# QualityMinds/cistgcn

Measured on AMD Instinct MI355X. Metric: sequences/sec (fwd+bwd) H3.6M 22-joint 50->25, higher is better.
Workload: dtype f32; 1 GPU; cistgcn64_b256_t50_v22; C=64, per_gpu_batch=256, global_batch=256, T_in=50, T_out=25, V=22, parallelism=dp1, graph=True, graph_branches=True, capture_kept=median, mixed_batches=False

## Files before the change

cistgcn_amd/csrc/stgcn_domain_planes.hip:

```cpp
#include "cg_common.h"
#include "stgcn_domain.h"
#include <stdlib.h>

HIP_DYNAMIC_SHARED(unsigned char, cg_dyn_lds)

typedef float cg_f32x4 __attribute__((vector_size(16)));
typedef float cg_f32x2 __attribute__((vector_size(8)));

#define CG_DOMP_THREADS 256
#define CG_DOMP_NW (CG_DOMP_THREADS / 64)

__device__ __forceinline__ int cg_domp_swz(int o) { const int h = o >> 1; return (h & 3) | ((h & 4) << 1); }

template <int VW>
__device__ __forceinline__ void cg_domp_ld(const float* __restrict__ p, bool ok, float (&v)[VW]) {
  if constexpr (VW == 4) {
    cg_f32x4 t = cg_f32x4{0.f, 0.f, 0.f, 0.f};
    if (ok) t = *reinterpret_cast<const cg_f32x4*>(p);
#pragma unroll
    for (int i = 0; i < VW; ++i) v[i] = t[i];
  } else if constexpr (VW == 2) {
    cg_f32x2 t = cg_f32x2{0.f, 0.f};
    if (ok) t = *reinterpret_cast<const cg_f32x2*>(p);
#pragma unroll
    for (int i = 0; i < VW; ++i) v[i] = t[i];
  } else {
    v[0] = ok ? p[0] : 0.f;
  }
}
template <int VW>
__device__ __forceinline__ void cg_domp_st(float* __restrict__ p, const float (&v)[VW]) {
  if constexpr (VW == 4) *reinterpret_cast<cg_f32x4*>(p) = cg_f32x4{v[0], v[1], v[2], v[3]};
  else if constexpr (VW == 2) *reinterpret_cast<cg_f32x2*>(p) = cg_f32x2{v[0], v[1]};
  else p[0] = v[0];
}

template <int DOMAIN>
__device__ __forceinline__ void cg_domp_split(const CgDomP& g, int p, int& grp, int& j) {
  const int t = (int)cg_div((unsigned)p, g.magicV), v = p - t * g.V;
  if (DOMAIN == 0) { grp = v; j = t; } else { grp = t; j = v; }
}

template <int DOMAIN, int VW>
__device__ __forceinline__ void cg_domp_mix_planes(const CgDomP& g, const float* __restrict__ xb, long long cs, int Cin, int KS,
                                                   const float* sW, int WS, float* sZ, int pbeg, int pend, int jshift) {
  const int lane = threadIdx.x & 63, wave = __builtin_amdgcn_readfirstlane(threadIdx.x >> 6), l15 = lane & 15, slot = lane >> 4;
  const int nunits = (pend - pbeg + 16 * VW - 1) / (16 * VW);
  const float* wrow = sW + l15 * WS + slot;
  for (int u = wave; u < nunits; u += CG_DOMP_NW) {
    const int p0 = pbeg + u * 16 * VW + VW * l15;
    const bool pok = p0 < pend;
    const float* xp = xb + p0 + (long long)slot * cs;
    cg_f32x4 acc[VW];
#pragma unroll
    for (int i = 0; i < VW; ++i) acc[i] = cg_f32x4{0.f, 0.f, 0.f, 0.f};
    float xa[4][VW], xc[4][VW];
    auto ld = [&](int k0, float (&xv)[4][VW]) {
#pragma unroll
      for (int s = 0; s < 4; ++s) cg_domp_ld<VW>(xp + (long long)(4 * (k0 + s)) * cs, pok && 4 * (k0 + s) + slot < Cin, xv[s]);
    };
    auto mm = [&](int k0, const float (&xv)[4][VW]) {
#pragma unroll
      for (int s = 0; s < 4; ++s) {
        if (k0 + s >= KS) break;
        const float a = wrow[4 * (k0 + s)];
#pragma unroll
        for (int i = 0; i < VW; ++i) acc[i] = __builtin_amdgcn_mfma_f32_16x16x4f32(a, xv[s][i], acc[i], 0, 0, 0);
      }
    };
    ld(0, xa);
    for (int k0 = 0; k0 < KS; k0 += 8) {
      if (k0 + 4 < KS) ld(k0 + 4, xc);
      mm(k0, xa);
      if (k0 + 4 < KS) {
        if (k0 + 8 < KS) ld(k0 + 8, xa);
        mm(k0 + 4, xc);
      }
    }
    if (pok) {
#pragma unroll
      for (int i = 0; i < VW; ++i) {
        int grp, j;
        cg_domp_split<DOMAIN>(g, p0 + i, grp, j);
        float* dst = sZ + grp * g.GSTR + (j - jshift) + 4 * slot * g.JS;
#pragma unroll
        for (int r = 0; r < 4; ++r) dst[r * g.JS] = acc[i][r];
      }
    }
  }
}

template <int DOMAIN, int VW, int VWB, int NL>
__global__ __launch_bounds__(CG_DOMP_THREADS, 2) void cg_stgcn_planes_fwd_kernel(const float* __restrict__ x, const float* __restrict__ adj,
                                                                 const float* __restrict__ W, const float* __restrict__ bias,
                                                                 float* __restrict__ y, double* __restrict__ ystats, CgDomP g) {
  float* sZ = reinterpret_cast<float*>(cg_dyn_lds);
  float* sW = sZ + g.zfloats;
  double* sStat = reinterpret_cast<double*>(sW + 16 * g.WS);
  const int tid = threadIdx.x, lane = tid & 63, wave = __builtin_amdgcn_readfirstlane(tid >> 6), l15 = lane & 15, slot = lane >> 4;
  const int xcd = blockIdx.x & 7, s = blockIdx.x >> 3;
  const int sb = s / g.NOC, oc = s - sb * g.NOC, b = sb * 8 + xcd;
  if (b >= g.B) return;
  const int o0 = oc * 16;

  for (int e = tid; e < 16 * g.WS; e += CG_DOMP_THREADS) {
    const int o = e / g.WS, c = e - o * g.WS;
    sW[e] = (o0 + o < g.Cout && c < g.Cin) ? W[(long long)(o0 + o) * g.Cin + c] : 0.f;
  }
  if (tid < 32) sStat[tid] = 0.0;
  __syncthreads();

  cg_domp_mix_planes<DOMAIN, VW>(g, x + (long long)b * g.Cin * g.TV, g.TV, g.Cin, g.KS, sW, g.WS, sZ, 0, g.TV, 0);
  __syncthreads();

  const int J = g.J;
  float bv[4];
#pragma unroll
  for (int r = 0; r < 4; ++r) { const int co = o0 + 4 * slot + r; bv[r] = (bias && co < g.Cout) ? bias[co] : 0.f; }
  double st1[4] = {0.0, 0.0, 0.0, 0.0}, st2[4] = {0.0, 0.0, 0.0, 0.0};
  for (int gi = wave; gi < g.NG; gi += CG_DOMP_NW) {
    float gs1[4] = {0.f, 0.f, 0.f, 0.f}, gs2[4] = {0.f, 0.f, 0.f, 0.f};
    const float* ag = adj + ((long long)b * g.NG + gi) * J * J;
    float* zs = sZ + gi * g.GSTR;
    const float* za = zs + l15 * g.JS + slot;
    cg_f32x4 acc[NL * VWB];
#pragma unroll
    for (int i = 0; i < NL * VWB; ++i) acc[i] = cg_f32x4{0.f, 0.f, 0.f, 0.f};
    float ba[4][NL][VWB], bc[4][NL][VWB];
    auto ld = [&](int k0, float (&v)[4][NL][VWB]) {
#pragma unroll
      for (int s2 = 0; s2 < 4; ++s2) {
        const int jr = 4 * (k0 + s2) + slot;
#pragma unroll
        for (int m = 0; m < NL; ++m) {
          const int q0 = (m * 16 + l15) * VWB;
          cg_domp_ld<VWB>(ag + (long long)jr * J + q0, jr < J && q0 < J, v[s2][m]);
        }
      }
    };
    auto mm = [&](int k0, const float (&v)[4][NL][VWB]) {
#pragma unroll
      for (int s2 = 0; s2 < 4; ++s2) {
        if (k0 + s2 >= g.JSTEPS) break;
        const int jr = 4 * (k0 + s2) + slot;
        const float a = jr < J ? za[4 * (k0 + s2)] : 0.f;
#pragma unroll
        for (int m = 0; m < NL; ++m)
#pragma unroll
          for (int i = 0; i < VWB; ++i) acc[m * VWB + i] = __builtin_amdgcn_mfma_f32_16x16x4f32(a, v[s2][m][i], acc[m * VWB + i], 0, 0, 0);
      }
    };
    ld(0, ba);
    for (int k0 = 0; k0 < g.JSTEPS; k0 += 8) {
      if (k0 + 4 < g.JSTEPS) ld(k0 + 4, bc);
      mm(k0, ba);
// ... 372 lines not shown
      cg_f32x4 c0 = cg_f32x4{0.f, 0.f, 0.f, 0.f};
      const float* ap = sdZ + l15 * XS + 4 * slot;
      const float* bp = sX + (16 * wct + l15) * XS + 4 * slot;
      for (int kc = wks; kc < NPT; kc += nks) {
        cg_f32x4 a0 = *reinterpret_cast<const cg_f32x4*>(ap + 16 * kc);
        const cg_f32x4 b0 = *reinterpret_cast<const cg_f32x4*>(bp + 16 * kc);
        if (16 * kc + 16 > Pn) {
#pragma unroll
          for (int s2 = 0; s2 < 4; ++s2) a0[s2] = (16 * kc + 4 * slot + s2 < Pn) ? a0[s2] : 0.f;
        }
#pragma unroll
        for (int s2 = 0; s2 < 4; ++s2) c0 = __builtin_amdgcn_mfma_f32_16x16x4f32(a0[s2], b0[s2], c0, 0, 0, 0);
      }
      if (wks == 0) dWhold = c0;
      else *reinterpret_cast<cg_f32x4*>(sPart + ((wave - MTc) * 64 + lane) * 4) = c0;
    }
    {
      const int ct = wave % MTc;
      const float* ap = sW + slot * WS + 16 * ct + l15;
      float aw[4];
#pragma unroll
      for (int st = 0; st < 4; ++st) aw[st] = ap[4 * st * WS];
#pragma unroll
      for (int i = 0; i < NDX; ++i) {
        const int id = wave + CG_DOMPB_NW * i;
        if (id < ndx) {
          const float* bp = sdZ + slot * XS + 16 * (id / MTc) + l15;
#pragma unroll
          for (int st = 0; st < 4; ++st) dxacc[i] = __builtin_amdgcn_mfma_f32_16x16x4f32(aw[st], bp[4 * st * XS], dxacc[i], 0, 0, 0);
        }
        if ((i & 3) == 3) __builtin_amdgcn_sched_barrier(0);
      }
    }
  }

  const int l15 = l15_, slot = slot_;
  CG_STAMP();
  __syncthreads();
  CG_STAMP();
  dw_flush(g.NOC - 1);
#pragma unroll
  for (int i = 0; i < NDX; ++i) {
    const int id = wave + CG_DOMPB_NW * i;
    if (id < ndx) {
      const int pt = id / MTc, ct = id - pt * MTc;
      float* dst = sX + (16 * ct + 4 * slot) * XS + 16 * pt + l15;
      if (16 * pt + l15 < Pn) {
#pragma unroll
        for (int r = 0; r < 4; ++r) dst[r * XS] = dxacc[i][r];
      }
    }
  }
#pragma unroll
  for (int a = 0; a < NJW; ++a) {
    const int v = wave + CG_DOMPB_NW * a;
    if (v < V) {
#pragma unroll
      for (int qc = 0; qc < 4; ++qc) {
        const int q = 16 * qc + l15;
        if (qc < NQC && q < T) {
          float* db_ = dadj + (((long long)b * V + v) * T + t0) * T;
#pragma unroll
          for (int r = 0; r < 4; ++r) {
            const int t = 4 * slot + r;
            if (t < TCn) db_[t * T + q] = dAacc[a][qc][r];
          }
        }
      }
    }
  }
  __syncthreads();
  {
    float* dxb = dx + (long long)b * Cin * TV + (long long)t0 * V;
    const int nvp = Pn / VWP;
    for (int c0 = 4 * wave; c0 < Cin; c0 += 4 * CG_DOMPB_NW) {
      float xr[8][VWP];
#pragma unroll
      for (int u = 0; u < 8; ++u) {
        const int c = c0 + (u >> 1), i = lane + 64 * (u & 1);
        if (c < Cin && i < nvp) {
          if constexpr (VWP == 4) {
            const cg_f32x4 t = *reinterpret_cast<const cg_f32x4*>(sX + c * XS + i * VWP);
#pragma unroll
            for (int jj = 0; jj < VWP; ++jj) xr[u][jj] = t[jj];
          } else {
#pragma unroll
            for (int jj = 0; jj < VWP; ++jj) xr[u][jj] = sX[c * XS + i * VWP + jj];
          }
        }
      }
#pragma unroll
      for (int u = 0; u < 8; ++u) {
        const int c = c0 + (u >> 1), i = lane + 64 * (u & 1);
        if (c < Cin && i < nvp) cg_domp_st<VWP>(dxb + ((long long)c * TV + i * VWP), xr[u]);
      }
    }
  }
  CG_STAMP();
  CG_STAMP_END();
}

static int cg_domp_up(int v, int m) { return (v + m - 1) / m * m; }

int cg_domp_geom(CgDomP& g, int B, int Cin, int Cout, int T, int V, int domain) {
  if (B <= 0 || Cin <= 0 || Cout <= 0 || T <= 0 || V <= 0 || (domain != 0 && domain != 1)) return CG_ESHAPE;
  g.B = B; g.Cin = Cin; g.Cout = Cout; g.T = T; g.V = V; g.TV = T * V;
  g.NG = domain == 1 ? T : V;
  g.J = domain == 1 ? V : T;
  if (g.J > 64 || Cin > 128 || (long long)T * V > (1 << 20)) return CG_ESHAPE;
  g.JS = g.J + ((2 - g.J) & 3);
  g.GSTR = 16 * g.JS + 2;
  g.NOC = (Cout + 15) / 16;
  g.KS = (Cin + 3) / 4;
  g.WS = 4 * cg_domp_up(g.KS, 4) + 2;
  g.JSTEPS = (g.J + 3) / 4;
  g.zfloats = cg_domp_up(g.NG * g.GSTR + 16, 4);
  g.VW = (g.TV % 4 == 0) ? 4 : (g.TV % 2 == 0) ? 2 : 1;
  if (g.J <= 16) { g.VWB = 1; g.NL = 1; }
  else if (g.J <= 32) { if (g.J % 2 == 0) { g.VWB = 2; g.NL = 1; } else { g.VWB = 1; g.NL = 2; } }
  else { if (g.J % 4 == 0) { g.VWB = 4; g.NL = 1; } else if (g.J % 2 == 0) { g.VWB = 2; g.NL = 2; } else { g.VWB = 1; g.NL = 4; } }
  g.magicV = cg_div_magic(V);
  g.magicNQ = cg_div_magic(g.TV / g.VW);
  return CG_OK;
}

size_t cg_domp_fwd_lds_bytes(const CgDomP& g) { return ((size_t)g.zfloats + 16 * (size_t)g.WS) * sizeof(float) + 32 * sizeof(double); }

int cg_domp_fwd_launch(const float* x, const float* adj, const float* W, const float* bias, float* y, double* ystats,
                       int B, int Cin, int Cout, int T, int V, int domain, hipStream_t stream) {
  CgDomP g;
  int st = cg_domp_geom(g, B, Cin, Cout, T, V, domain);
  if (st != CG_OK) return st;
  const size_t lds = cg_domp_fwd_lds_bytes(g);
  if (lds > 160 * 1024 - 512) return CG_ESHAPE;
  dim3 grid((unsigned)(8 * ((B + 7) / 8) * g.NOC)), block(CG_DOMP_THREADS);
#define CG_DOMP_FWD(D, VW_, VWB_, NL_)                                                                                              \
  if (domain == D && g.VW == VW_ && g.VWB == VWB_ && g.NL == NL_) {                                                               \
    hipError_t e = cg_lds_limit((const void*)cg_stgcn_planes_fwd_kernel<D, VW_, VWB_, NL_>,                                \
                                       lds);                                       \
    if (e != hipSuccess) return (int)e;                                                                                             \
    hipLaunchKernelGGL((cg_stgcn_planes_fwd_kernel<D, VW_, VWB_, NL_>), grid, block, lds, stream, x, adj, W, bias, y, ystats, g);   \
    return cg_launch_status();                                                                                                      \
  }
  CG_DOMP_FWD(0, 4, 2, 2)
  CG_DOMP_FWD(0, 2, 2, 2)
  CG_DOMP_FWD(0, 4, 1, 1)
  CG_DOMP_FWD(0, 2, 1, 1)
  CG_DOMP_FWD(1, 4, 2, 1)
  CG_DOMP_FWD(1, 2, 1, 2)
#undef CG_DOMP_FWD
  return CG_ESHAPE;
}

#define CG_DOMPT_THREADS 512
#define CG_DOMPT_NW 8

template <int VWP, int VWA>
__global__ __launch_bounds__(CG_DOMPT_THREADS, 2) void cg_stgcn_planes_bwd_time_kernel(const float* __restrict__ x, const float* __restrict__ adj,
                                                                       const float* __restrict__ W, const float* __restrict__ dy,
                                                                       float* __restrict__ dx, float* __restrict__ dadj,
                                                                       float* __restrict__ ws, int replicas, CgDomP g) {
  const int T = g.T, V = g.V, Cin = g.Cin, Cout = g.Cout, XS = g.XS, WS = g.WS, CinR = g.CinR, CoR = 16 * g.NOC;
  const int DR = max(CinR, CoR);
  float* sX = reinterpret_cast<float*>(cg_dyn_lds);
  float* sDY = sX + CinR * XS;
  float* sZ = sDY + DR * XS;
  float* sW = sZ + CoR * XS;
  float* sdb = sW + CoR * WS;
  const int tid = threadIdx.x, lane = tid & 63, wave = __builtin_amdgcn_readfirstlane(tid >> 6), l15 = lane & 15, slot = lane >> 4;
  const int xcd = blockIdx.x & 7, sidx = blockIdx.x >> 3;
  const int sb = sidx / g.NTC, tc = sidx - sb * g.NTC, b = sb * 8 + xcd;
  if (b >= g.B) return;
  const int t0 = tc * g.TC, TCn = min(g.TC, T - t0), Pn = TCn * V, NPT = (Pn + 15) / 16;
  const long long TV = g.TV;
  const int MTc = CinR / 16, MTo = g.NOC;

  int nst = 0; (void)nst;
  CG_STAMP();
  {
    const int nvp = Pn / VWP;
    const float* xb = x + (long long)b * Cin * TV + (long long)t0 * V;
    const float* yb = dy + (long long)b * Cout * TV + (long long)t0 * V;
    const int rows = Cin + Cout;
    float buf[16][VWP];
    const int r0 = 16 * wave;
#pragma unroll
    for (int u = 0; u < 16; ++u) {
      const int r = r0 + u;
      const float* src = r < Cin ? xb + (long long)r * TV : yb + (long long)(r - Cin) * TV;
      cg_domp_ld<VWP>(src + lane * VWP, r < rows && lane < nvp, buf[u]);
    }
    const int padc = XS - Pn, nrow = CinR + DR + CoR;
    for (int e = tid; e < nrow * padc; e += CG_DOMPT_THREADS) {
      const int r = e / padc, c = e - r * padc;
      sX[r * XS + Pn + c] = 0.f;
    }
    for (int e = tid; e < (CinR - Cin) * Pn; e += CG_DOMPT_THREADS) sX[Cin * XS + (e / Pn) * XS + e % Pn] = 0.f;
    for (int e = tid; e < (DR - Cout) * Pn; e += CG_DOMPT_THREADS) sDY[Cout * XS + (e / Pn) * XS + e % Pn] = 0.f;
    for (int e = tid; e < CoR * (WS + 1); e += CG_DOMPT_THREADS) sW[e] = 0.f;
    __syncthreads();
    CG_STAMP();
#pragma unroll
    for (int u = 0; u < 16; ++u) {
      const int r = r0 + u;
      float* dst = r < Cin ? sX + r * XS : sDY + (r - Cin) * XS;
      if (r < rows && lane < nvp) {
#pragma unroll
        for (int jj = 0; jj < VWP; ++jj) dst[lane * VWP + jj] = buf[u][jj];
      }
    }
    for (int e = tid; e < Cout * Cin; e += CG_DOMPT_THREADS) {
      const int o = e / Cin, c = e - o * Cin;
      sW[o * WS + c] = W[e];
    }
  }
  CG_STAMP();
  __syncthreads();
  CG_STAMP();

  {
    const int OP = (MTo + 1) / 2, nun = OP * NPT;
    for (int u = wave; u < nun; u += CG_DOMPT_NW) {
      const int pt = u / OP, op = u - pt * OP, ot0 = 2 * op, ot1 = ot0 + 1 < MTo ? ot0 + 1 : ot0;
      cg_f32x4 a0 = cg_f32x4{0.f, 0.f, 0.f, 0.f}, a1 = a0;
      const float* ap0 = sW + (16 * ot0 + l15) * WS + slot;
      const float* ap1 = sW + (16 * ot1 + l15) * WS + slot;
      const float* bp = sX + slot * XS + 16 * pt + l15;
      float f0[12], f1[12];
      auto ld = [&](int k0, float (&f)[12]) {
#pragma unroll
        for (int s2 = 0; s2 < 4; ++s2) { f[s2] = ap0[4 * (k0 + s2)]; f[4 + s2] = ap1[4 * (k0 + s2)]; f[8 + s2] = bp[4 * (k0 + s2) * XS]; }
      };
      auto mm = [&](const float (&f)[12]) {
#pragma unroll
        for (int s2 = 0; s2 < 4; ++s2) {
          a0 = __builtin_amdgcn_mfma_f32_16x16x4f32(f[s2], f[8 + s2], a0, 0, 0, 0);
          a1 = __builtin_amdgcn_mfma_f32_16x16x4f32(f[4 + s2], f[8 + s2], a1, 0, 0, 0);
        }
      };
      const int KS4 = CinR / 4;
      ld(0, f0);
      for (int k0 = 0; k0 < KS4; k0 += 8) {
        if (k0 + 4 < KS4) ld(k0 + 4, f1);
        mm(f0);
        if (k0 + 4 < KS4) {
          if (k0 + 8 < KS4) ld(k0 + 8, f0);
          mm(f1);
        }
      }
      if (16 * pt + l15 < Pn) {
#pragma unroll
        for (int r = 0; r < 4; ++r) {
          sZ[(16 * ot0 + 4 * slot + r) * XS + 16 * pt + l15] = a0[r];
          if (ot1 != ot0) sZ[(16 * ot1 + 4 * slot + r) * XS + 16 * pt + l15] = a1[r];
        }
      }
    }
  }
  CG_STAMP();
  __syncthreads();
  CG_STAMP();

  float dbw[4] = {0.f, 0.f, 0.f, 0.f};
  for (int tl = wave; tl < TCn; tl += CG_DOMPT_NW) {
    const int pb = tl * V;
    const int NVT = (V + 15) / 16;
    const float* at = adj + (((long long)b * T + t0 + tl) * V) * V;
    float bv[2][2][4];
#pragma unroll
    for (int kc = 0; kc < 2; ++kc)
#pragma unroll
      for (int j = 0; j < 2; ++j) {
        const int v = 16 * j + l15, w0 = 16 * kc + 4 * slot;
#pragma unroll
        for (int s0 = 0; s0 < 4; s0 += VWA) {
          float tmp[VWA];
          cg_domp_ld<VWA>(at + v * V + w0 + s0, kc < NVT && j < NVT && v < V && w0 + s0 < V, tmp);
#pragma unroll
          for (int q = 0; q < VWA; ++q) bv[kc][j][s0 + q] = tmp[q];
        }
      }
    {
      cg_f32x4 acc[2][2];
#pragma unroll
      for (int i = 0; i < 2; ++i)
#pragma unroll
        for (int j = 0; j < 2; ++j) acc[i][j] = cg_f32x4{0.f, 0.f, 0.f, 0.f};
      const float* zp = sZ + slot * XS + pb + l15;
      const float* yp = sDY + slot * XS + pb + l15;
      float fa[16], fb[16];
      auto ld = [&](int k0, float (&f)[16]) {
#pragma unroll
        for (int s2 = 0; s2 < 4; ++s2)
#pragma unroll
          for (int i = 0; i < 2; ++i) { f[4 * s2 + i] = zp[4 * (k0 + s2) * XS + 16 * i]; f[4 * s2 + 2 + i] = yp[4 * (k0 + s2) * XS + 16 * i]; }
      };
      auto mm = [&](const float (&f)[16]) {
#pragma unroll
        for (int s2 = 0; s2 < 4; ++s2)
#pragma unroll
          for (int i = 0; i < 2; ++i)
#pragma unroll
            for (int j = 0; j < 2; ++j)
              if (i < NVT && j < NVT) acc[i][j] = __builtin_amdgcn_mfma_f32_16x16x4f32(f[4 * s2 + i], f[4 * s2 + 2 + j], acc[i][j], 0, 0, 0);
      };
      const int KS4 = CoR / 4;
      ld(0, fa);
      for (int k0 = 0; k0 < KS4; k0 += 8) {
        if (k0 + 4 < KS4) ld(k0 + 4, fb);
        mm(fa);
        if (k0 + 4 < KS4) {
          if (k0 + 8 < KS4) ld(k0 + 8, fa);
          mm(fb);
        }
      }
      float* da = dadj + (((long long)b * T + t0 + tl) * V) * V;
#pragma unroll
      for (int i = 0; i < 2; ++i)
#pragma unroll
        for (int j = 0; j < 2; ++j) {
          const int w = 16 * j + l15;
          if (i < NVT && j < NVT && w < V) {
#pragma unroll
            for (int r = 0; r < 4; ++r) {
              const int v = 16 * i + 4 * slot + r;
              if (v < V) da[v * V + w] = acc[i][j][r];
            }
          }
        }
    }
    {
      cg_f32x4 acc[4][2];
#pragma unroll
      for (int i = 0; i < 4; ++i)
#pragma unroll
        for (int j = 0; j < 2; ++j) acc[i][j] = cg_f32x4{0.f, 0.f, 0.f, 0.f};
      float dbp[4] = {0.f, 0.f, 0.f, 0.f};
#pragma unroll
      for (int kc = 0; kc < 2; ++kc) {
        if (kc < NVT) {
          const int w0 = 16 * kc + 4 * slot;
          float av[4][4];
#pragma unroll
          for (int i = 0; i < 4; ++i)
#pragma unroll
            for (int s2 = 0; s2 < 4; ++s2) av[i][s2] = (i < MTo && w0 + s2 < V) ? sDY[(16 * i + l15) * XS + pb + w0 + s2] : 0.f;
#pragma unroll
          for (int s2 = 0; s2 < 4; ++s2)
#pragma unroll
            for (int i = 0; i < 4; ++i) {
              dbp[i] += av[i][s2];
#pragma unroll
              for (int j = 0; j < 2; ++j)
                if (i < MTo && j < NVT) acc[i][j] = __builtin_amdgcn_mfma_f32_16x16x4f32(av[i][s2], bv[kc][j][s2], acc[i][j], 0, 0, 0);
            }
        }
      }
#pragma unroll
      for (int i = 0; i < 4; ++i)
#pragma unroll
        for (int j = 0; j < 2; ++j) {
          const int v = 16 * j + l15;
          if (i < MTo && j < NVT && v < V) {
#pragma unroll
            for (int r = 0; r < 4; ++r) sZ[(16 * i + 4 * slot + r) * XS + pb + v] = acc[i][j][r];
          }
        }
#pragma unroll
      for (int i = 0; i < 4; ++i) dbw[i] += dbp[i];
    }
  }
#pragma unroll
  for (int i = 0; i < 4; ++i) {
    float sdbp = dbw[i];
    sdbp += __shfl_xor(sdbp, 16, 64);
    sdbp += __shfl_xor(sdbp, 32, 64);
    if (i < MTo && slot == 0) atomicAdd(&sdb[16 * i + l15], sdbp);
  }
  CG_STAMP();
  __syncthreads();
  CG_STAMP();

  {
    const int CP = (MTc + 1) / 2, nun = CP * NPT;
    for (int u = wave; u < nun; u += CG_DOMPT_NW) {
      const int pt = u / CP, cp = u - pt * CP, ct0 = 2 * cp, ct1 = ct0 + 1 < MTc ? ct0 + 1 : ct0;
      cg_f32x4 a0 = cg_f32x4{0.f, 0.f, 0.f, 0.f}, a1 = a0;
      const float* ap0 = sW + slot * WS + 16 * ct0 + l15;
      const float* ap1 = sW + slot * WS + 16 * ct1 + l15;
      const float* bp = sZ + slot * XS + 16 * pt + l15;
      float f0[12], f1[12];
      auto ld = [&](int k0, float (&f)[12]) {
#pragma unroll
        for (int s2 = 0; s2 < 4; ++s2) { f[s2] = ap0[4 * (k0 + s2) * WS]; f[4 + s2] = ap1[4 * (k0 + s2) * WS]; f[8 + s2] = bp[4 * (k0 + s2) * XS]; }
      };
      auto mm = [&](const float (&f)[12]) {
#pragma unroll
        for (int s2 = 0; s2 < 4; ++s2) {
          a0 = __builtin_amdgcn_mfma_f32_16x16x4f32(f[s2], f[8 + s2], a0, 0, 0, 0);
          a1 = __builtin_amdgcn_mfma_f32_16x16x4f32(f[4 + s2], f[8 + s2], a1, 0, 0, 0);
        }
      };
      const int KS4 = CoR / 4;
      ld(0, f0);
      for (int k0 = 0; k0 < KS4; k0 += 8) {
        if (k0 + 4 < KS4) ld(k0 + 4, f1);
        mm(f0);
        if (k0 + 4 < KS4) {
          if (k0 + 8 < KS4) ld(k0 + 8, f0);
          mm(f1);
        }
      }
      if (16 * pt + l15 < Pn) {
#pragma unroll
        for (int r = 0; r < 4; ++r) {
          sDY[(16 * ct0 + 4 * slot + r) * XS + 16 * pt + l15] = a0[r];
          if (ct1 != ct0) sDY[(16 * ct1 + 4 * slot + r) * XS + 16 * pt + l15] = a1[r];
        }
      }
    }
    float* wsr = ws + (long long)(blockIdx.x % replicas) * ((long long)Cout * Cin + Cout);
    const int CP2 = (MTc + 1) / 2;
    for (int u = wave; u < MTo * CP2; u += CG_DOMPT_NW) {
      const int ot = u / CP2, cp = u - ot * CP2, ct0 = 2 * cp, ct1 = ct0 + 1 < MTc ? ct0 + 1 : ct0;
      cg_f32x4 a0 = cg_f32x4{0.f, 0.f, 0.f, 0.f}, a1 = a0;
      const float* ap = sZ + (16 * ot + l15) * XS + 4 * slot;
      const float* bp0 = sX + (16 * ct0 + l15) * XS + 4 * slot;
      const float* bp1 = sX + (16 * ct1 + l15) * XS + 4 * slot;
      float fa[12], fb[12];
      auto ld = [&](int kc, float (&f)[12]) {
#pragma unroll
        for (int s2 = 0; s2 < 4; ++s2) {
          const bool ok = 16 * kc + 4 * slot + s2 < Pn;
          f[s2] = ok ? ap[16 * kc + s2] : 0.f; f[4 + s2] = bp0[16 * kc + s2]; f[8 + s2] = bp1[16 * kc + s2];
        }
      };
      auto mm = [&](const float (&f)[12]) {
#pragma unroll
        for (int s2 = 0; s2 < 4; ++s2) {
          a0 = __builtin_amdgcn_mfma_f32_16x16x4f32(f[s2], f[4 + s2], a0, 0, 0, 0);
          a1 = __builtin_amdgcn_mfma_f32_16x16x4f32(f[s2], f[8 + s2], a1, 0, 0, 0);
        }
      };
      ld(0, fa);
      for (int kc = 0; kc < NPT; kc += 2) {
        if (kc + 1 < NPT) ld(kc + 1, fb);
        mm(fa);
        if (kc + 1 < NPT) {
          if (kc + 2 < NPT) ld(kc + 2, fa);
          mm(fb);
        }
      }
#pragma unroll
      for (int r = 0; r < 4; ++r) {
        const int co = 16 * ot + 4 * slot + r;
        if (co < Cout && 16 * ct0 + l15 < Cin) atomicAdd(&wsr[(long long)co * Cin + 16 * ct0 + l15], a0[r]);
        if (ct1 != ct0 && co < Cout && 16 * ct1 + l15 < Cin) atomicAdd(&wsr[(long long)co * Cin + 16 * ct1 + l15], a1[r]);
      }
    }
    if (tid < Cout) atomicAdd(&wsr[(long long)Cout * Cin + tid], sdb[tid]);
  }
  CG_STAMP();
  __syncthreads();
  CG_STAMP();
  {
    float* dxb = dx + (long long)b * Cin * TV + (long long)t0 * V;
    const int nvp = Pn / VWP;
    for (int r0 = 8 * wave; r0 < Cin; r0 += 8 * CG_DOMPT_NW) {
      float buf[8][VWP];
#pragma unroll
      for (int u = 0; u < 8; ++u) {
        const int r = r0 + u;
        if (r < Cin && lane < nvp) {
#pragma unroll
          for (int jj = 0; jj < VWP; ++jj) buf[u][jj] = sDY[r * XS + lane * VWP + jj];
        }
      }
#pragma unroll
      for (int u = 0; u < 8; ++u) {
        const int r = r0 + u;
        if (r < Cin && lane < nvp) cg_domp_st<VWP>(dxb + ((long long)r * TV + lane * VWP), buf[u]);
      }
    }
  }
  CG_STAMP();
  CG_STAMP_END();
}

static int cg_domp_xs(int p) { int xs = cg_domp_up(p, 4); return (xs % 8 == 4) ? xs : xs + 4; }

int cg_domp_bwd_geom(CgDomP& g, int B, int Cin, int Cout, int T, int V) {
  int st = cg_domp_geom(g, B, Cin, Cout, T, V, 0);
  if (st != CG_OK) return st;
  if (Cin > 64 || T > 64) return CG_ESHAPE;
  g.CinR = cg_domp_up(Cin, 16);
  g.YS = 16; g.GZ = 16 * 16 + 1; g.GY = 16 * 16 + 1;
  g.zfl = cg_domp_up(V * g.GZ, 4); g.yfl = cg_domp_up(V * g.GY, 4);
  g.WS = cg_domp_up(g.WS, 2);
  const size_t limit = 160 * 1024 - 1024;
  for (int ntc = (T + 15) / 16; ntc <= T; ++ntc) {
    const int tc0 = (T + ntc - 1) / ntc;
    int best = 0, best_al = 0;
    for (int tc = tc0; tc <= 16 && tc <= tc0 + 2; ++tc) {
      if ((long long)(ntc - 1) * tc >= T) continue;
      const int last = T - (ntc - 1) * tc;
      const int al = ((tc * V) % 4 == 0 && (last * V) % 4 == 0 && g.TV % 4 == 0) ? 4 : ((tc * V) % 2 == 0 && (last * V) % 2 == 0 && g.TV % 2 == 0) ? 2 : 1;
      const int xs = cg_domp_xs(tc * V);
      const int dzfl = 16 * xs > g.yfl ? 16 * xs : g.yfl;
      const size_t bytes = ((size_t)g.CinR * xs + dzfl + g.zfl + g.yfl + 16 * (size_t)g.WS + CG_DOMPB_NW * 256 + 64) * sizeof(float);
      if (bytes > limit || (g.CinR / 16) * ((tc * V + 15) / 16) > CG_DOMPB_NDX * CG_DOMPB_NW || tc * V > 128 * al) continue;
      if (al > best_al) { best = tc; best_al = al; }
    }
    if (best) {
      g.NTC = ntc; g.TC = best; g.VWP = best_al;
      g.XS = cg_domp_xs(best * V);
      g.dzfl = 16 * g.XS > g.yfl ? 16 * g.XS : g.yfl;
      g.bwd_floats = g.CinR * g.XS + g.dzfl + g.zfl + g.yfl + 16 * g.WS + CG_DOMPB_NW * 256 + 64;
      const int lastq = T - 16 * ((T + 15) / 16 - 1);
      g.VWY = (g.TV % 4 == 0 && (lastq * V) % 4 == 0) ? 4 : (g.TV % 2 == 0 && (lastq * V) % 2 == 0) ? 2 : 1;
      g.VWA = T % 4 == 0 ? 4 : T % 2 == 0 ? 2 : 1;
      return CG_OK;
    }
  }
  return CG_ESHAPE;
}

int cg_domp_bwd_launch(const float* x, const float* adj, const float* W, const float* dy, float* dx, float* dadj, float* ws,
                       int replicas, int B, int Cin, int Cout, int T, int V, int domain, hipStream_t stream) {
  if (domain != 0) return CG_ESHAPE;
  CgDomP g;
  int st = cg_domp_bwd_geom(g, B, Cin, Cout, T, V);
  if (st != CG_OK) return st;
  const size_t lds = (size_t)g.bwd_floats * sizeof(float);
  const int njw = (V + CG_DOMPB_NW - 1) / CG_DOMPB_NW;
  dim3 grid((unsigned)(8 * ((B + 7) / 8) * g.NTC)), block(CG_DOMPB_THREADS);
  const int pfn = (16 * V / g.VWY + 31) / 32;
  if (CG_DOMPB_NW % (g.CinR / 16) != 0 || 16 * g.WS > 3 * CG_DOMPB_THREADS) return CG_ESHAPE;
  const int ndxw = ((g.CinR / 16) * ((g.TC * V + 15) / 16) + CG_DOMPB_NW - 1) / CG_DOMPB_NW;
#define CG_DOMP_BWD(VWP_, VWY_, VWA_, NJW_, PF_, NDX_)                                                                             \
  if (g.VWP == VWP_ && g.VWY == VWY_ && g.VWA == VWA_ && njw <= NJW_ && pfn <= PF_ && ndxw <= NDX_) {                             \
    hipError_t e = cg_lds_limit((const void*)cg_stgcn_planes_bwd_kernel<VWP_, VWY_, VWA_, NJW_, PF_, NDX_>,                \
                                       lds);                                      \
    if (e != hipSuccess) return (int)e;                                                                                            \
    hipLaunchKernelGGL((cg_stgcn_planes_bwd_kernel<VWP_, VWY_, VWA_, NJW_, PF_, NDX_>), grid, block, lds, stream, x, adj, W, dy,  \
                       dx, dadj, ws, replicas, g);                                                                                 \
    return cg_launch_status();                                                                                                     \
  }
  CG_DOMP_BWD(4, 4, 2, 3, 3, 10)
  CG_DOMP_BWD(2, 2, 2, 4, 7, 6)
#undef CG_DOMP_BWD
  return CG_ESHAPE;
}

int cg_domp_bwd_time_launch(const float* x, const float* adj, const float* W, const float* dy, float* dx, float* dadj, float* ws,
                            int replicas, int B, int Cin, int Cout, int T, int V, hipStream_t stream) {
  CgDomP g;
  int st = cg_domp_geom(g, B, Cin, Cout, T, V, 1);
  if (st != CG_OK) return st;
  if (Cin > 64 || Cout > 64 || V > 32) return CG_ESHAPE;
  g.CinR = cg_domp_up(Cin, 16);
  const int CoR = 16 * g.NOC;
  g.WS = cg_domp_up(g.CinR, 4) + 2;
  g.TC = CG_DOMPT_NW;
  if (g.TC > T) g.TC = T;
  g.NTC = (T + g.TC - 1) / g.TC;
  const int last = T - (g.NTC - 1) * g.TC;
  g.VWP = ((g.TC * V) % 4 == 0 && (last * V) % 4 == 0 && g.TV % 4 == 0) ? 4 : ((g.TC * V) % 2 == 0 && (last * V) % 2 == 0 && g.TV % 2 == 0) ? 2 : 1;
  if (g.TC * V > 64 * g.VWP || Cin + Cout > 16 * CG_DOMPT_NW) return CG_ESHAPE;
  g.VWA = V % 4 == 0 ? 4 : V % 2 == 0 ? 2 : 1;
  g.XS = g.TC * V + ((2 - g.TC * V) & 3);
  if (g.XS < cg_domp_up(g.TC * V, 16)) g.XS += 4 * ((cg_domp_up(g.TC * V, 16) - g.XS + 3) / 4);
  g.bwd_floats = (g.CinR + (g.CinR > CoR ? g.CinR : CoR) + CoR) * g.XS + CoR * (g.WS + 1) + 64;
  const size_t lds = (size_t)g.bwd_floats * sizeof(float);
  if (lds > 160 * 1024 - 512) return CG_ESHAPE;
  dim3 grid((unsigned)(8 * ((B + 7) / 8) * g.NTC)), block(CG_DOMPT_THREADS);
#define CG_DOMP_BWDT(VWP_, VWA_)                                                                                                   \
  if (g.VWP == VWP_ && g.VWA == VWA_) {                                                                                            \
    hipError_t e = cg_lds_limit((const void*)cg_stgcn_planes_bwd_time_kernel<VWP_, VWA_>,                                   \
                                       lds);                                      \
    if (e != hipSuccess) return (int)e;                                                                                            \
    hipLaunchKernelGGL((cg_stgcn_planes_bwd_time_kernel<VWP_, VWA_>), grid, block, lds, stream, x, adj, W, dy, dx, dadj, ws,       \
                       replicas, g);                                                                                               \
    return cg_launch_status();                                                                                                     \
  }
  CG_DOMP_BWDT(4, 2)
  CG_DOMP_BWDT(2, 1)
#undef CG_DOMP_BWDT
  return CG_ESHAPE;
}
```

Baseline: 15220 sequences/sec.

## Double block to 1024 threads, split adjoint/dz work per frame across wave pairs

The backward-time kernel goes from 512 to 1024 threads (16 waves) while keeping an 8-frame time chunk. Each frame now gets two waves, one computing the adjacency gradient and one computing the dz product. Weight staging is restructured so W is loaded into registers early and written into padded LDS in one pass, removing a barrier. A tail-splitting work dealer spreads leftover MFMA tiles across more waves, and the adjacency loads are hoisted ahead of the prologue barrier. The cost is fewer blocks resident per CU (launch bounds drop the min-2-blocks hint), more registers held across phases, and an extra barrier.

```diff
diff --git a/cistgcn_amd/csrc/stgcn_domain_planes.hip b/cistgcn_amd/csrc/stgcn_domain_planes.hip
--- a/cistgcn_amd/csrc/stgcn_domain_planes.hip
+++ b/cistgcn_amd/csrc/stgcn_domain_planes.hip
@@ -1,6 +1,7 @@
 #include "cg_common.h"
 #include "stgcn_domain.h"
 #include <stdlib.h>
+#include <type_traits>
 
 HIP_DYNAMIC_SHARED(unsigned char, cg_dyn_lds)
 
@@ -679,11 +680,32 @@
   return CG_ESHAPE;
 }
 
-#define CG_DOMPT_THREADS 512
-#define CG_DOMPT_NW 8
+#define CG_DOMPT_THREADS 1024
+#define CG_DOMPT_NW 16
+#define CG_DOMPT_TC 8
+#define CG_DOMPT_ROWS 8
+#define CG_DOMPT_WV 5
+static_assert(2 * CG_DOMPT_TC == CG_DOMPT_NW, "P2: two waves per frame of the chunk");
+
+template <class F>
+__device__ __forceinline__ void cg_dompt_deal(int wave, int nun, int NP, int MT, F&& fn) {
+  const int rounds = nun / CG_DOMPT_NW, rem = nun - rounds * CG_DOMPT_NW;
+  const bool split = 2 * rem <= CG_DOMPT_NW;
+  for (int it = 0; it <= rounds; ++it) {
+    int u, half = 0;
+    bool single = false;
+    if (it < rounds) u = wave + it * CG_DOMPT_NW;
+    else if (split) { if (wave >= 2 * rem) break; u = rounds * CG_DOMPT_NW + (wave >> 1); half = wave & 1; single = true; }
+    else { if (wave >= rem) break; u = rounds * CG_DOMPT_NW + wave; }
+    const int outer = u / NP, t0 = 2 * (u - outer * NP) + half;
+    if (t0 >= MT) continue;
+    if (!single && t0 + 1 < MT) fn(outer, t0, std::true_type{});
+    else fn(outer, t0, std::false_type{});
+  }
+}
 
 template <int VWP, int VWA>
-__global__ __launch_bounds__(CG_DOMPT_THREADS, 2) void cg_stgcn_planes_bwd_time_kernel(const float* __restrict__ x, const float* __restrict__ adj,
+__global__ __launch_bounds__(CG_DOMPT_THREADS) void cg_stgcn_planes_bwd_time_kernel(const float* __restrict__ x, const float* __restrict__ adj,
                                                                        const float* __restrict__ W, const float* __restrict__ dy,
                                                                        float* __restrict__ dx, float* __restrict__ dadj,
                                                                        float* __restrict__ ws, int replicas, CgDomP g) {
@@ -702,6 +724,13 @@
   const long long TV = g.TV;
   const int MTc = CinR / 16, MTo = g.NOC;
 
+  const int tl = wave >> 1;
+  const int pb = tl * V;
+  const int NVT = (V + 15) / 16;
+  const bool wave_da = tl < TCn && !(wave & 1), wave_dz = tl < TCn && (wave & 1);
+  const float* at = adj + (((long long)b * T + t0 + tl) * V) * V;
+  float bv[2][2][4];
+
   int nst = 0; (void)nst;
   CG_STAMP();
   {
@@ -709,14 +738,33 @@
     const float* xb = x + (long long)b * Cin * TV + (long long)t0 * V;
     const float* yb = dy + (long long)b * Cout * TV + (long long)t0 * V;
     const int rows = Cin + Cout;
-    float buf[16][VWP];
-    const int r0 = 16 * wave;
-#pragma unroll
-    for (int u = 0; u < 16; ++u) {
+    float buf[CG_DOMPT_ROWS][VWP];
+    const int r0 = CG_DOMPT_ROWS * wave;
+#pragma unroll
+    for (int u = 0; u < CG_DOMPT_ROWS; ++u) {
       const int r = r0 + u;
       const float* src = r < Cin ? xb + (long long)r * TV : yb + (long long)(r - Cin) * TV;
       cg_domp_ld<VWP>(src + lane * VWP, r < rows && lane < nvp, buf[u]);
     }
+    float wv[CG_DOMPT_WV];
+#pragma unroll
+    for (int i = 0; i < CG_DOMPT_WV; ++i) {
+      const int e = tid + i * CG_DOMPT_THREADS, o = e / WS, c = e - o * WS;
+      wv[i] = (o < Cout && c < Cin) ? W[o * Cin + c] : 0.f;
+    }
+#pragma unroll
+    for (int kc = 0; kc < 2; ++kc)
+#pragma unroll
+      for (int j = 0; j < 2; ++j) {
+        const int v = 16 * j + l15, w0 = 16 * kc + 4 * slot;
+#pragma unroll
+        for (int s0 = 0; s0 < 4; s0 += VWA) {
+          float tmp[VWA];
+          cg_domp_ld<VWA>(at + v * V + w0 + s0, wave_dz && kc < NVT && j < NVT && v < V && w0 + s0 < V, tmp);
+#pragma unroll
+          for (int q = 0; q < VWA; ++q) bv[kc][j][s0 + q] = tmp[q];
+        }
+      }
     const int padc = XS - Pn, nrow = CinR + DR + CoR;
     for (int e = tid; e < nrow * padc; e += CG_DOMPT_THREADS) {
       const int r = e / padc, c = e - r * padc;
@@ -724,11 +772,14 @@
     }
     for (int e = tid; e < (CinR - Cin) * Pn; e += CG_DOMPT_THREADS) sX[Cin * XS + (e / Pn) * XS + e % Pn] = 0.f;
     for (int e = tid; e < (DR - Cout) * Pn; e += CG_DOMPT_THREADS) sDY[Cout * XS + (e / Pn) * XS + e % Pn] = 0.f;
-    for (int e = tid; e < CoR * (WS + 1); e += CG_DOMPT_THREADS) sW[e] = 0.f;
-    __syncthreads();
     CG_STAMP();
 #pragma unroll
-    for (int u = 0; u < 16; ++u) {
+    for (int i = 0; i < CG_DOMPT_WV; ++i) {
+      const int e = tid + i * CG_DOMPT_THREADS;
+      if (e < CoR * (WS + 1)) sW[e] = wv[i];
+    }
+#pragma unroll
+    for (int u = 0; u < CG_DOMPT_ROWS; ++u) {
       const int r = r0 + u;
       float* dst = r < Cin ? sX + r * XS : sDY + (r - Cin) * XS;
       if (r < rows && lane < nvp) {
@@ -736,33 +787,34 @@
         for (int jj = 0; jj < VWP; ++jj) dst[lane * VWP + jj] = buf[u][jj];
       }
     }
-    for (int e = tid; e < Cout * Cin; e += CG_DOMPT_THREADS) {
-      const int o = e / Cin, c = e - o * Cin;
-      sW[o * WS + c] = W[e];
-    }
   }
   CG_STAMP();
   __syncthreads();
   CG_STAMP();
 
   {
-    const int OP = (MTo + 1) / 2, nun = OP * NPT;
-    for (int u = wave; u < nun; u += CG_DOMPT_NW) {
-      const int pt = u / OP, op = u - pt * OP, ot0 = 2 * op, ot1 = ot0 + 1 < MTo ? ot0 + 1 : ot0;
+    const int OP = (MTo + 1) / 2;
+    cg_dompt_deal(wave, OP * NPT, OP, MTo, [&](int pt, int ot0, auto two_) {
+      constexpr bool TWO = decltype(two_)::value;
+      const int ot1 = ot0 + 1;
       cg_f32x4 a0 = cg_f32x4{0.f, 0.f, 0.f, 0.f}, a1 = a0;
       const float* ap0 = sW + (16 * ot0 + l15) * WS + slot;
-      const float* ap1 = sW + (16 * ot1 + l15) * WS + slot;
+      const float* ap1 = ap0 + 16 * WS;
       const float* bp = sX + slot * XS + 16 * pt + l15;
       float f0[12], f1[12];
       auto ld = [&](int k0, float (&f)[12]) {
 #pragma unroll
-        for (int s2 = 0; s2 < 4; ++s2) { f[s2] = ap0[4 * (k0 + s2)]; f[4 + s2] = ap1[4 * (k0 + s2)]; f[8 + s2] = bp[4 * (k0 + s2) * XS]; }
+        for (int s2 = 0; s2 < 4; ++s2) {
+          f[s2] = ap0[4 * (k0 + s2)];
+          if constexpr (TWO) f[4 + s2] = ap1[4 * (k0 + s2)];
+          f[8 + s2] = bp[4 * (k0 + s2) * XS];
+        }
       };
       auto mm = [&](const float (&f)[12]) {
 #pragma unroll
         for (int s2 = 0; s2 < 4; ++s2) {
           a0 = __builtin_amdgcn_mfma_f32_16x16x4f32(f[s2], f[8 + s2], a0, 0, 0, 0);
-          a1 = __builtin_amdgcn_mfma_f32_16x16x4f32(f[4 + s2], f[8 + s2], a1, 0, 0, 0);
+          if constexpr (TWO) a1 = __builtin_amdgcn_mfma_f32_16x16x4f32(f[4 + s2], f[8 + s2], a1, 0, 0, 0);
         }
       };
       const int KS4 = CinR / 4;
@@ -779,34 +831,22 @@
 #pragma unroll
         for (int r = 0; r < 4; ++r) {
           sZ[(16 * ot0 + 4 * slot + r) * XS + 16 * pt + l15] = a0[r];
-          if (ot1 != ot0) sZ[(16 * ot1 + 4 * slot + r) * XS + 16 * pt + l15] = a1[r];
-        }
-      }
-    }
+          if constexpr (TWO) sZ[(16 * ot1 + 4 * slot + r) * XS + 16 * pt + l15] = a1[r];
+        }
+      }
+    });
   }
   CG_STAMP();
   __syncthreads();
   CG_STAMP();
 
-  float dbw[4] = {0.f, 0.f, 0.f, 0.f};
-  for (int tl = wave; tl < TCn; tl += CG_DOMPT_NW) {
-    const int pb = tl * V;
-    const int NVT = (V + 15) / 16;
-    const float* at = adj + (((long long)b * T + t0 + tl) * V) * V;
-    float bv[2][2][4];
-#pragma unroll
-    for (int kc = 0; kc < 2; ++kc)
-#pragma unroll
-      for (int j = 0; j < 2; ++j) {
-        const int v = 16 * j + l15, w0 = 16 * kc + 4 * slot;
-#pragma unroll
-        for (int s0 = 0; s0 < 4; s0 += VWA) {
-          float tmp[VWA];
-          cg_domp_ld<VWA>(at + v * V + w0 + s0, kc < NVT && j < NVT && v < V && w0 + s0 < V, tmp);
-#pragma unroll
-          for (int q = 0; q < VWA; ++q) bv[kc][j][s0 + q] = tmp[q];
-        }
-      }
+  cg_f32x4 dz[4][2];
+  float dbp[4] = {0.f, 0.f, 0.f, 0.f};
+#pragma unroll
+  for (int i = 0; i < 4; ++i)
+#pragma unroll
+    for (int j = 0; j < 2; ++j) dz[i][j] = cg_f32x4{0.f, 0.f, 0.f, 0.f};
+  if (wave_da) {
     {
       cg_f32x4 acc[2][2];
 #pragma unroll
@@ -856,13 +896,9 @@
           }
         }
     }
+  }
+  if (wave_dz) {
     {
-      cg_f32x4 acc[4][2];
-#pragma unroll
-      for (int i = 0; i < 4; ++i)
-#pragma unroll
-        for (int j = 0; j < 2; ++j) acc[i][j] = cg_f32x4{0.f, 0.f, 0.f, 0.f};
-      float dbp[4] = {0.f, 0.f, 0.f, 0.f};
 #pragma unroll
       for (int kc = 0; kc < 2; ++kc) {
         if (kc < NVT) {
@@ -879,53 +915,61 @@
               dbp[i] += av[i][s2];
 #pragma unroll
               for (int j = 0; j < 2; ++j)
-                if (i < MTo && j < NVT) acc[i][j] = __builtin_amdgcn_mfma_f32_16x16x4f32(av[i][s2], bv[kc][j][s2], acc[i][j], 0, 0, 0);
+                if (i < MTo && j < NVT) dz[i][j] = __builtin_amdgcn_mfma_f32_16x16x4f32(av[i][s2], bv[kc][j][s2], dz[i][j], 0, 0, 0);
             }
         }
       }
-#pragma unroll
-      for (int i = 0; i < 4; ++i)
-#pragma unroll
-        for (int j = 0; j < 2; ++j) {
-          const int v = 16 * j + l15;
-          if (i < MTo && j < NVT && v < V) {
-#pragma unroll
-            for (int r = 0; r < 4; ++r) sZ[(16 * i + 4 * slot + r) * XS + pb + v] = acc[i][j][r];
-          }
-        }
-#pragma unroll
-      for (int i = 0; i < 4; ++i) dbw[i] += dbp[i];
-    }
-  }
-#pragma unroll
-  for (int i = 0; i < 4; ++i) {
-    float sdbp = dbw[i];
-    sdbp += __shfl_xor(sdbp, 16, 64);
-    sdbp += __shfl_xor(sdbp, 32, 64);
-    if (i < MTo && slot == 0) atomicAdd(&sdb[16 * i + l15], sdbp);
+    }
   }
   CG_STAMP();
   __syncthreads();
   CG_STAMP();
+  if (wave_dz) {
+#pragma unroll
+    for (int i = 0; i < 4; ++i)
+#pragma unroll
+      for (int j = 0; j < 2; ++j) {
+        const int v = 16 * j + l15;
+        if (i < MTo && j < NVT && v < V) {
+#pragma unroll
+          for (int r = 0; r < 4; ++r) sZ[(16 * i + 4 * slot + r) * XS + pb + v] = dz[i][j][r];
+        }
+      }
+#pragma unroll
+    for (int i = 0; i < 4; ++i) {
+      float sdbp = dbp[i];
+      sdbp += __shfl_xor(sdbp, 16, 64);
+      sdbp += __shfl_xor(sdbp, 32, 64);
+      if (i < MTo && slot == 0) atomicAdd(&sdb[16 * i + l15], sdbp);
+    }
+  }
+  CG_STAMP();
+  __syncthreads();
+  CG_STAMP();
 
   {
-    const int CP = (MTc + 1) / 2, nun = CP * NPT;
-    for (int u = wave; u < nun; u += CG_DOMPT_NW) {
-      const int pt = u / CP, cp = u - pt * CP, ct0 = 2 * cp, ct1 = ct0 + 1 < MTc ? ct0 + 1 : ct0;
+    const int CP = (MTc + 1) / 2;
+    cg_dompt_deal(wave, CP * NPT, CP, MTc, [&](int pt, int ct0, auto two_) {
+      constexpr bool TWO = decltype(two_)::value;
+      const int ct1 = ct0 + 1;
       cg_f32x4 a0 = cg_f32x4{0.f, 0.f, 0.f, 0.f}, a1 = a0;
       const float* ap0 = sW + slot * WS + 16 * ct0 + l15;
-      const float* ap1 = sW + slot * WS + 16 * ct1 + l15;
+      const float* ap1 = ap0 + 16;
       const float* bp = sZ + slot * XS + 16 * pt + l15;
       float f0[12], f1[12];
       auto ld = [&](int k0, float (&f)[12]) {
 #pragma unroll
-        for (int s2 = 0; s2 < 4; ++s2) { f[s2] = ap0[4 * (k0 + s2) * WS]; f[4 + s2] = ap1[4 * (k0 + s2) * WS]; f[8 + s2] = bp[4 * (k0 + s2) * XS]; }
+        for (int s2 = 0; s2 < 4; ++s2) {
+          f[s2] = ap0[4 * (k0 + s2) * WS];
+          if constexpr (TWO) f[4 + s2] = ap1[4 * (k0 + s2) * WS];
+          f[8 + s2] = bp[4 * (k0 + s2) * XS];
+        }
       };
       auto mm = [&](const float (&f)[12]) {
 #pragma unroll
         for (int s2 = 0; s2 < 4; ++s2) {
           a0 = __builtin_amdgcn_mfma_f32_16x16x4f32(f[s2], f[8 + s2], a0, 0, 0, 0);
-          a1 = __builtin_amdgcn_mfma_f32_16x16x4f32(f[4 + s2], f[8 + s2], a1, 0, 0, 0);
+          if constexpr (TWO) a1 = __builtin_amdgcn_mfma_f32_16x16x4f32(f[4 + s2], f[8 + s2], a1, 0, 0, 0);
         }
       };
       const int KS4 = CoR / 4;
@@ -942,31 +986,33 @@
 #pragma unroll
         for (int r = 0; r < 4; ++r) {
           sDY[(16 * ct0 + 4 * slot + r) * XS + 16 * pt + l15] = a0[r];
-          if (ct1 != ct0) sDY[(16 * ct1 + 4 * slot + r) * XS + 16 * pt + l15] = a1[r];
-        }
-      }
-    }
+          if constexpr (TWO) sDY[(16 * ct1 + 4 * slot + r) * XS + 16 * pt + l15] = a1[r];
+        }
+      }
+    });
     float* wsr = ws + (long long)(blockIdx.x % replicas) * ((long long)Cout * Cin + Cout);
-    const int CP2 = (MTc + 1) / 2;
-    for (int u = wave; u < MTo * CP2; u += CG_DOMPT_NW) {
-      const int ot = u / CP2, cp = u - ot * CP2, ct0 = 2 * cp, ct1 = ct0 + 1 < MTc ? ct0 + 1 : ct0;
+    cg_dompt_deal(wave, MTo * CP, CP, MTc, [&](int ot, int ct0, auto two_) {
+      constexpr bool TWO = decltype(two_)::value;
+      const int ct1 = ct0 + 1;
       cg_f32x4 a0 = cg_f32x4{0.f, 0.f, 0.f, 0.f}, a1 = a0;
       const float* ap = sZ + (16 * ot + l15) * XS + 4 * slot;
       const float* bp0 = sX + (16 * ct0 + l15) * XS + 4 * slot;
-      const float* bp1 = sX + (16 * ct1 + l15) * XS + 4 * slot;
+      const float* bp1 = bp0 + 16 * XS;
       float fa[12], fb[12];
       auto ld = [&](int kc, float (&f)[12]) {
 #pragma unroll
         for (int s2 = 0; s2 < 4; ++s2) {
           const bool ok = 16 * kc + 4 * slot + s2 < Pn;
-          f[s2] = ok ? ap[16 * kc + s2] : 0.f; f[4 + s2] = bp0[16 * kc + s2]; f[8 + s2] = bp1[16 * kc + s2];
+          f[s2] = ok ? ap[16 * kc + s2] : 0.f;
+          f[4 + s2] = bp0[16 * kc + s2];
+          if constexpr (TWO) f[8 + s2] = bp1[16 * kc + s2];
         }
       };
       auto mm = [&](const float (&f)[12]) {
 #pragma unroll
         for (int s2 = 0; s2 < 4; ++s2) {
           a0 = __builtin_amdgcn_mfma_f32_16x16x4f32(f[s2], f[4 + s2], a0, 0, 0, 0);
-          a1 = __builtin_amdgcn_mfma_f32_16x16x4f32(f[s2], f[8 + s2], a1, 0, 0, 0);
+          if constexpr (TWO) a1 = __builtin_amdgcn_mfma_f32_16x16x4f32(f[s2], f[8 + s2], a1, 0, 0, 0);
         }
       };
       ld(0, fa);
@@ -982,9 +1028,11 @@
       for (int r = 0; r < 4; ++r) {
         const int co = 16 * ot + 4 * slot + r;
         if (co < Cout && 16 * ct0 + l15 < Cin) atomicAdd(&wsr[(long long)co * Cin + 16 * ct0 + l15], a0[r]);
-        if (ct1 != ct0 && co < Cout && 16 * ct1 + l15 < Cin) atomicAdd(&wsr[(long long)co * Cin + 16 * ct1 + l15], a1[r]);
-      }
-    }
+        if constexpr (TWO) {
+          if (co < Cout && 16 * ct1 + l15 < Cin) atomicAdd(&wsr[(long long)co * Cin + 16 * ct1 + l15], a1[r]);
+        }
+      }
+    });
     if (tid < Cout) atomicAdd(&wsr[(long long)Cout * Cin + tid], sdb[tid]);
   }
   CG_STAMP();
@@ -993,10 +1041,10 @@
   {
     float* dxb = dx + (long long)b * Cin * TV + (long long)t0 * V;
     const int nvp = Pn / VWP;
-    for (int r0 = 8 * wave; r0 < Cin; r0 += 8 * CG_DOMPT_NW) {
-      float buf[8][VWP];
-#pragma unroll
-      for (int u = 0; u < 8; ++u) {
+    for (int r0 = 4 * wave; r0 < Cin; r0 += 4 * CG_DOMPT_NW) {
+      float buf[4][VWP];
+#pragma unroll
+      for (int u = 0; u < 4; ++u) {
         const int r = r0 + u;
         if (r < Cin && lane < nvp) {
 #pragma unroll
@@ -1004,7 +1052,7 @@
         }
       }
 #pragma unroll
-      for (int u = 0; u < 8; ++u) {
+      for (int u = 0; u < 4; ++u) {
         const int r = r0 + u;
         if (r < Cin && lane < nvp) cg_domp_st<VWP>(dxb + ((long long)r * TV + lane * VWP), buf[u]);
       }
@@ -1088,18 +1136,18 @@
   g.CinR = cg_domp_up(Cin, 16);
   const int CoR = 16 * g.NOC;
   g.WS = cg_domp_up(g.CinR, 4) + 2;
-  g.TC = CG_DOMPT_NW;
+  g.TC = CG_DOMPT_TC;
   if (g.TC > T) g.TC = T;
   g.NTC = (T + g.TC - 1) / g.TC;
   const int last = T - (g.NTC - 1) * g.TC;
   g.VWP = ((g.TC * V) % 4 == 0 && (last * V) % 4 == 0 && g.TV % 4 == 0) ? 4 : ((g.TC * V) % 2 == 0 && (last * V) % 2 == 0 && g.TV % 2 == 0) ? 2 : 1;
-  if (g.TC * V > 64 * g.VWP || Cin + Cout > 16 * CG_DOMPT_NW) return CG_ESHAPE;
+  if (g.TC * V > 64 * g.VWP || Cin + Cout > CG_DOMPT_ROWS * CG_DOMPT_NW) return CG_ESHAPE;
   g.VWA = V % 4 == 0 ? 4 : V % 2 == 0 ? 2 : 1;
   g.XS = g.TC * V + ((2 - g.TC * V) & 3);
   if (g.XS < cg_domp_up(g.TC * V, 16)) g.XS += 4 * ((cg_domp_up(g.TC * V, 16) - g.XS + 3) / 4);
   g.bwd_floats = (g.CinR + (g.CinR > CoR ? g.CinR : CoR) + CoR) * g.XS + CoR * (g.WS + 1) + 64;
   const size_t lds = (size_t)g.bwd_floats * sizeof(float);
-  if (lds > 160 * 1024 - 512) return CG_ESHAPE;
+  if (lds > 160 * 1024 - 512 || CoR * (g.WS + 1) > CG_DOMPT_WV * CG_DOMPT_THREADS) return CG_ESHAPE;
   dim3 grid((unsigned)(8 * ((B + 7) / 8) * g.NTC)), block(CG_DOMPT_THREADS);
 #define CG_DOMP_BWDT(VWP_, VWA_)                                                                                                   \
   if (g.VWP == VWP_ && g.VWA == VWA_) {                                                                                            \
```

Result: no change. 15310 sequences/sec, median of 6 (+0.6%).
